# gabrielfnayres/new-vit

Measured on AMD Instinct MI355X. Metric: volumes_per_sec_mst_dinov2_fwd, higher is better.
Workload: dtype bf16; 1 GPU; MST-DINOv2 (DinoV2ClassifierSlice, ViT-S/14) forward, 4 volumes/GPU of 64x512x512 bf16 zero-padded to 518x518 (N=1370 tokens/slice); global_batch_volumes=4, slices=64, parallelism=single GPU, weights=synthetic (mst.synth seed 2), random init of the reference architecture

## Files before the change

new-vit_amd/csrc/k_gemm16_wreg.hip:

```cpp
#include <cstdlib>

#include "mst_common.h"

namespace {

constexpr int KD = GEMM16_WREG_TILE.bk, BN = GEMM16_WREG_TILE.bn, CH = GEMM16_WREG_TILE.bm;
constexpr int ROWB = KD * 2;
constexpr int SLOT = CH * ROWB;
constexpr int WREG_NSLOT = 4;
constexpr int NSLOT = WREG_NSLOT;
constexpr int STG_PITCH = ROWB + 16;
constexpr int STG_BYTES = CH * STG_PITCH;
constexpr int STG_OFF = NSLOT * SLOT;
constexpr int LDS_BYTES = STG_OFF + 2 * STG_BYTES;
constexpr int NKT = KD / 32;
constexpr int PPW = SLOT / 1024 / 8;
static_assert(NSLOT == 4, "the counted vmcnt table below is written for three chunks in flight");

#define WREG_RD(dst, base, imm) asm volatile("ds_read_b128 %0, %1 offset:%2" : "=v"(dst) : "v"(base), "n"(imm) : "memory")

template <typename T, bool BLK>
__global__ __launch_bounds__(512) __attribute__((amdgpu_waves_per_eu(2, 2))) void gemm16_wreg_kernel(
    const T* __restrict__ A, int64_t lda, const T* __restrict__ W, int64_t ldw, const float* __restrict__ bias, T* __restrict__ C,
    int64_t ldc, int M, int N, float col_scale, int scale_cols, int nchunks) {
    typedef typename V8<T>::type vec8;
    typedef __attribute__((ext_vector_type(4))) T out4;
    extern __shared__ __attribute__((aligned(16))) char smem[];
    const int lane = threadIdx.x & 63;
    const int wave = __builtin_amdgcn_readfirstlane(threadIdx.x >> 6);
    const int frow = lane & 15, kq = lane >> 4;

    const int xcd = blockIdx.x & 7, g = blockIdx.x >> 3, G = gridDim.x >> 3;
    const int tiles_n = N / BN;
    const int nt = g % tiles_n, jcu = g / tiles_n;
    const int c_nt = (G - nt + tiles_n - 1) / tiles_n;
    const int per_xcd = (nchunks + 7) >> 3;
    const int lo = xcd * per_xcd;
    const int hi = lo + per_xcd < nchunks ? lo + per_xcd : nchunks;
    const int n0 = nt * BN + wave * 48;
    const float cs = nt * BN < scale_cols ? col_scale : 1.f;

    vec8 w[3][NKT];
#pragma unroll
    for (int t = 0; t < 3; ++t) {
        const T* wr = W + (int64_t)(n0 + 12 * (frow >> 2) + 4 * t + (frow & 3)) * ldw + kq * 8;
#pragma unroll
        for (int kt = 0; kt < NKT; ++kt) w[t][kt] = *reinterpret_cast<const vec8*>(wr + kt * 32);
    }
    f32x4 b[3];
#pragma unroll
    for (int t = 0; t < 3; ++t) {
        b[t] = (f32x4){0.f, 0.f, 0.f, 0.f};
        if (bias) b[t] = *reinterpret_cast<const f32x4*>(bias + n0 + 12 * kq + 4 * t);
    }
#pragma unroll
    for (int t = 0; t < 3; ++t) {
        asm volatile("" : "+v"(b[t]));
#pragma unroll
        for (int kt = 0; kt < NKT; ++kt) asm volatile("" : "+v"(w[t][kt]));
    }

    unsigned dma_off[PPW];
#pragma unroll
    for (int u = 0; u < PPW; ++u) {
        const int o = (wave * PPW + u) * 1024 + lane * 16;
        const int r = o / ROWB;
        dma_off[u] = BLK ? (unsigned)o : (unsigned)(r * (int)lda * 2 + ((((o % ROWB) >> 4) ^ (r & 15)) << 4));
    }
    const int64_t chunk_bytes = BLK ? (int64_t)SLOT : (int64_t)CH * lda * 2;
    auto issue_piece = [&](int chunk, int slot, int u) {
        const char* base = reinterpret_cast<const char*>(A) + (int64_t)chunk * chunk_bytes;
        unsigned off = dma_off[u];
        const int valid = M - chunk * CH;
        if (!BLK && valid < CH) {
            const int o = (wave * PPW + u) * 1024 + lane * 16;
            int r = o / ROWB;
            const int ck = ((o % ROWB) >> 4) ^ (r & 15);
            r = r < valid ? r : valid - 1;
            off = (unsigned)(r * (int)lda * 2 + ck * 16);
        }
        __builtin_amdgcn_global_load_lds(GLB_PTR(base + off), LDS_PTR(smem + slot * SLOT + (wave * PPW + u) * 1024), 16, 0, 0);
    };

    int rb[4];
#pragma unroll
    for (int j = 0; j < 4; ++j) rb[j] = BLK ? (kq >> 1) * 1024 + (frow + 32 * (kq & 1)) * 16 : frow * ROWB + (((4 * j + kq) ^ frow) << 4);
    const int put_off = frow * STG_PITCH + wave * 96 + kq * 24;
    int fl_lds[3];
    unsigned fl_glb[3];
    int fl_row[3];
#pragma unroll
    for (int j = 0; j < 3; ++j) {
        const int q = lane + 64 * j;
        fl_row[j] = wave * 4 + q / 48;
        fl_lds[j] = fl_row[j] * STG_PITCH + (q % 48) * 16;
        fl_glb[j] = (unsigned)(fl_row[j] * (int)ldc * 2 + nt * BN * 2 + (q % 48) * 16);
    }
    f32x4 acc[2][3];
    auto put = [&](int it) {
        char* stg = smem + STG_OFF + (it & 1) * STG_BYTES + put_off;
#pragma unroll
        for (int mt = 0; mt < 2; ++mt)
#pragma unroll
            for (int t = 0; t < 3; ++t) {
                out4 pk;
#pragma unroll
                for (int i = 0; i < 4; ++i) pk[i] = (T)(acc[mt][t][i] * cs);
                *reinterpret_cast<out4*>(stg + mt * 16 * STG_PITCH + t * 8) = pk;
            }
    };
    auto flush_piece = [&](int chunk, int it, int j) {
        const char* stg = smem + STG_OFF + (it & 1) * STG_BYTES;
        char* cb = reinterpret_cast<char*>(C) + (int64_t)chunk * CH * ldc * 2;
        const int valid = M - chunk * CH;
        const u32x4 v = *reinterpret_cast<const u32x4*>(stg + fl_lds[j]);
        if (valid >= CH || fl_row[j] < valid) {
            __builtin_nontemporal_store(v, reinterpret_cast<u32x4*>(cb + fl_glb[j]));
        }
    };
    auto flush = [&](int chunk, int it) {
#pragma unroll
        for (int j = 0; j < 3; ++j) flush_piece(chunk, it, j);
    };

    int c = lo + jcu;
    if (c >= hi) return;
#pragma unroll
    for (int d = 0; d < NSLOT - 1; ++d)
        if (c + d * c_nt < hi) {
#pragma unroll
            for (int u = 0; u < PPW; ++u) issue_piece(c + d * c_nt, d, u);
        }

    int prev = -1, last_it = 0;
    for (int it = 0; c < hi; c += c_nt, ++it) {
        if (c + 2 * c_nt < hi) {
            if (it <= 1) asm volatile("s_waitcnt vmcnt(6)" ::: "memory");
            else if (it == 2) asm volatile("s_waitcnt vmcnt(9)" ::: "memory");
            else asm volatile("s_waitcnt vmcnt(12)" ::: "memory");
        } else {
            asm volatile("s_waitcnt vmcnt(0)" ::: "memory");
        }
        asm volatile("s_waitcnt lgkmcnt(0)\n\ts_barrier" ::: "memory");
        if (prev >= 0) flush(prev, it - 1);

        const int slot = it % NSLOT;
        const int nxt = c + (NSLOT - 1) * c_nt, nslot = (it + NSLOT - 1) % NSLOT;
        const bool more = nxt < hi;
        int rbs[4];
#pragma unroll
        for (int j = 0; j < 4; ++j) rbs[j] = rb[j] + slot * SLOT;
#pragma unroll
        for (int mt = 0; mt < 2; ++mt)
#pragma unroll
            for (int t = 0; t < 3; ++t) acc[mt][t] = b[t];

        u32x4 a[2][2];
        WREG_RD(a[0][0], rbs[0], 0);
        if constexpr (BLK) WREG_RD(a[0][1], rbs[0], 256);
        else WREG_RD(a[0][1], rbs[0], 16 * ROWB);
#pragma unroll
        for (int kt = 0; kt < NKT; ++kt) {
            const int cur = kt & 1;
            if (kt + 1 < NKT) {
                switch (kt + 1) {
#define WREG_NEXT(KN)                                                                  \
    case KN:                                                                           \
        if constexpr (BLK) {                                                           \
            WREG_RD(a[(KN) & 1][0], rbs[0], (KN) * 2048);                              \
            WREG_RD(a[(KN) & 1][1], rbs[0], (KN) * 2048 + 256);                        \
        } else {                                                                       \
            WREG_RD(a[(KN) & 1][0], rbs[(KN) & 3], ((KN) >> 2) * 256);                 \
            WREG_RD(a[(KN) & 1][1], rbs[(KN) & 3], 16 * ROWB + ((KN) >> 2) * 256);     \
        }                                                                              \
        break;
                    WREG_NEXT(1) WREG_NEXT(2) WREG_NEXT(3) WREG_NEXT(4) WREG_NEXT(5) WREG_NEXT(6)
                    WREG_NEXT(7) WREG_NEXT(8) WREG_NEXT(9) WREG_NEXT(10) WREG_NEXT(11)
#undef WREG_NEXT
                }
                asm volatile("s_waitcnt lgkmcnt(2)" : "+v"(a[cur][0]), "+v"(a[cur][1])::"memory");
            } else {
                asm volatile("s_waitcnt lgkmcnt(0)" : "+v"(a[cur][0]), "+v"(a[cur][1])::"memory");
            }
            const vec8 a0 = __builtin_bit_cast(vec8, a[cur][0]), a1 = __builtin_bit_cast(vec8, a[cur][1]);
#pragma unroll
            for (int t = 0; t < 3; ++t) {
                acc[0][t] = mfma16(w[t][kt], a0, acc[0][t]);
                acc[1][t] = mfma16(w[t][kt], a1, acc[1][t]);
            }
            if ((kt & 3) == 1) {
                __builtin_amdgcn_sched_barrier(0);
                if (more) issue_piece(nxt, nslot, kt >> 2);
                __builtin_amdgcn_sched_barrier(0);
            }
        }
        put(it);
        prev = c;
        last_it = it;
    }
    asm volatile("s_waitcnt lgkmcnt(0)\n\ts_barrier" ::: "memory");
    flush(prev, last_it);
}

template <typename T, bool BLK>
int launch_t(const gemm_args& g) {
    static mst_lds_once lds_once;
    auto kern = gemm16_wreg_kernel<T, BLK>;
    mst_allow_lds((const void*)kern, LDS_BYTES, &lds_once);
    const int nchunks = (int)((g.M + CH - 1) / CH);
    kern<<<dim3(mst_persistent_grid()), dim3(512), LDS_BYTES, g.s>>>((const T*)g.A, g.lda, (const T*)g.W, g.ldw, g.bias, (T*)g.C, g.ldc, (int)g.M,
                                                                      g.N, g.col_scale, g.scale_cols, nchunks);
    return mst_check_launch("gemm16_wreg");
}

}

int launch_gemm16_wreg(const gemm_args& g, int a_blocked) {
    if (a_blocked) {
        if (g.dt == MST_BF16) return launch_t<bf16_t, true>(g);
        if (g.dt == MST_F16) return launch_t<f16_t, true>(g);
    }
    if (g.dt == MST_BF16) return launch_t<bf16_t, false>(g);
    if (g.dt == MST_F16) return launch_t<f16_t, false>(g);
    mst_set_error("gemm16_wreg: bad operand dtype %d", g.dt);
    return MST_EINVAL;
}
```

new-vit_amd/mst/hip/__init__.py:

```python
from __future__ import annotations

import ctypes as C
import os
from pathlib import Path
from typing import Sequence, Optional, Tuple

import torch

_HERE = Path(__file__).resolve().parent
LIB_PATH = Path(os.environ.get("MST_HIP_LIB", _HERE / "libmst_hip.so"))

F32, F16, BF16, F8E4M3 = 0, 1, 2, 3
EPI_BIAS, EPI_BIAS_GELU, EPI_BIAS_RELU, EPI_RESIDUAL, EPI_RESIDUAL_RELU, EPI_BIAS_SWIGLU = 0, 1, 2, 3, 4, 5
FFN_MLP, FFN_SWIGLU = 0, 1
FUSION_TRANSFORMER, FUSION_LINEAR, FUSION_AVERAGE = 0, 1, 2

_DT = {torch.float32: F32, torch.float16: F16, torch.bfloat16: BF16}
TORCH_DT = {F32: torch.float32, F16: torch.float16, BF16: torch.bfloat16}
DT_NAMES = {"fp32": F32, "f32": F32, "float32": F32, "fp16": F16, "f16": F16, "float16": F16,
            "bf16": BF16, "bfloat16": BF16,
            "fp8": BF16, "f8": BF16, "fp8_e4m3": BF16}
FP8_NAMES = ("fp8", "f8", "fp8_e4m3")

_vp, _i, _i64, _f, _d, _sz = C.c_void_p, C.c_int, C.c_int64, C.c_float, C.c_double, C.c_size_t
# ... 117 lines not shown
    "mst_batchnorm_bwd_ordered": (_i, [_vp, _vp, _vp, _vp, _vp, _i64, _i, _vp, _vp, _vp, _vp, _sz, _vp]),
    "mst_col2im_nhwc_gather": (_i, [_vp, _i, _i, _i, _i, _i, _i, _i, _i, _i, _vp, _vp]),
    "mst_maxpool_bwd_nhwc_gather_workspace_bytes": (_sz, [_i, _i, _i, _i]),
    "mst_maxpool_bwd_nhwc_gather": (_i, [_vp, _vp, _i, _i, _i, _i, _vp, _vp, _sz, _vp]),
    "mst_pos_embed_interp_bwd_ordered_workspace_bytes": (_sz, [_i, _i, _i, _i]),
    "mst_pos_embed_interp_bwd_ordered": (_i, [_vp, _i, _i, _i, _i, _d, _vp, _vp, _sz, _vp]),
    "mst_znorm_ordered_workspace_bytes": (_sz, [_i64]),
    "mst_znorm_ordered": (_i, [_vp, _i64, _f, _f, _vp, _vp, _vp, _sz, _vp]),
    "mst_profiler_create": (_vp, []),
    "mst_profiler_destroy": (None, [_vp]),
    "mst_profiler_collect": (_i, [_vp, C.POINTER(C.c_double), C.POINTER(C.c_int64)]),
    "mst_kernel_kind_name": (C.c_char_p, [_i]),
}
K_COUNT = 10
ABI_VERSION = 300

_lib: Optional[C.CDLL] = None


def load() -> C.CDLL:
    global _lib
    if _lib is None:
        if not LIB_PATH.exists():
            raise RuntimeError(
                f"libmst_hip.so not found at {LIB_PATH}: build it with `python new-vit_amd/build.py` "
                "(hipcc --offload-arch=gfx950). There is no CPU / PyTorch fallback for the MST hot path.")
        lib = C.CDLL(str(LIB_PATH))
        for name, (res, args) in SIGNATURES.items():
            fn = getattr(lib, name)
            fn.restype, fn.argtypes = res, args
        if lib.mst_version() != ABI_VERSION:
            raise RuntimeError(f"{LIB_PATH} reports ABI version {lib.mst_version()}, this binding was written for {ABI_VERSION}: "
                               "rebuild with `python new-vit_amd/build.py --force`")
        _lib = lib
    return _lib


def last_error() -> str:
    return (load().mst_last_error() or b"").decode()


def _check(rc: int, what: str):
    if rc != 0:
        raise RuntimeError(f"{what} failed (status {rc}): {last_error()}")


def dt_of(t: torch.Tensor) -> int:
    try:
        return _DT[t.dtype]
    except KeyError:
        raise TypeError(f"unsupported dtype {t.dtype}") from None


def ptr(t: Optional[torch.Tensor]):
    return None if t is None else t.data_ptr()


def stream_of(t: torch.Tensor):
    return torch.cuda.current_stream(t.device).cuda_stream


def deterministic() -> bool:
    return torch.are_deterministic_algorithms_enabled()


def workspace(nbytes: int, device) -> Optional[torch.Tensor]:
    return torch.empty(int(nbytes), dtype=torch.uint8, device=device) if nbytes else None


def _call_ws(name: str, size_args, t: torch.Tensor, *args, sized_by: Optional[str] = None):
    lib = load()
    ws = workspace(getattr(lib, (sized_by or name) + "_workspace_bytes")(*size_args), t.device)
    _check(getattr(lib, name)(*args, ptr(ws), 0 if ws is None else ws.numel(), stream_of(t)), name)


def _dev(t: torch.Tensor, what: str):
    if not t.is_cuda:
        raise RuntimeError(f"{what}: tensor must live on a HIP device (got {t.device}); the MST kernels have no CPU path")
    if not t.is_contiguous():
        raise RuntimeError(f"{what}: tensor must be contiguous")


def layernorm(x: torch.Tensor, weight: torch.Tensor, bias: torch.Tensor, eps: float,
              out_dtype: torch.dtype = torch.float32) -> torch.Tensor:
    _dev(x, "layernorm")
    rows, cols = x.numel() // x.shape[-1], x.shape[-1]
    out = torch.empty(x.shape, dtype=out_dtype, device=x.device)
    _check(load().mst_layernorm(ptr(x), cols, ptr(weight), ptr(bias), ptr(out), _DT[out_dtype], cols, rows, cols,
                                eps, stream_of(x)), "mst_layernorm")
    return out


def gemm(a: torch.Tensor, w: torch.Tensor, bias: Optional[torch.Tensor], *, epilogue: int = EPI_BIAS,
         out: Optional[torch.Tensor] = None, out_dtype: Optional[torch.dtype] = None,
         gamma: Optional[torch.Tensor] = None, col_scale: float = 1.0, scale_cols: int = 0) -> torch.Tensor:
    _dev(a, "gemm")
    _dev(w, "gemm")
    M, K = a.shape
    N = w.shape[0]
    n_out = N // 2 if epilogue == EPI_BIAS_SWIGLU else N
    if out is None:
        out = torch.empty((M, n_out), dtype=out_dtype or a.dtype, device=a.device)
    _check(load().mst_gemm(ptr(a), dt_of(a), K, ptr(w), K, ptr(bias), ptr(out), dt_of(out), n_out, M, N, K, epilogue,
                           ptr(gamma), col_scale, scale_cols, stream_of(a)), "mst_gemm")
    return out


F8_MAX = 448.0


def quantize_weight_fp8(w: torch.Tensor) -> Tuple[torch.Tensor, float]:
    w = w.detach().to(torch.float32)
    amax = float(w.abs().max())
    scale = amax / F8_MAX if amax > 0 else 1.0
    q = (w / scale).clamp(-F8_MAX, F8_MAX).to(torch.float8_e4m3fn)
    return q.view(torch.uint8).contiguous(), scale


def quantize_fp8(x: torch.Tensor, amax: Optional[torch.Tensor] = None) -> Tuple[torch.Tensor, torch.Tensor]:
    _dev(x, "quantize_fp8")
    if amax is None:
        amax = torch.zeros(1, dtype=torch.float32, device=x.device)
    out = torch.empty(x.shape, dtype=torch.uint8, device=x.device)
    _check(load().mst_quantize_fp8(ptr(x), dt_of(x), x.numel(), ptr(amax), ptr(out), stream_of(x)), "mst_quantize_fp8")
    return out, amax


def gemm_fp8(a8: torch.Tensor, a_amax: torch.Tensor, w8: torch.Tensor, w_scale: float, bias: Optional[torch.Tensor], *,
             epilogue: int = EPI_BIAS, out: Optional[torch.Tensor] = None, out_dtype: torch.dtype = torch.float32,
             gamma: Optional[torch.Tensor] = None, col_scale: float = 1.0, scale_cols: int = 0,
             c_amax: Optional[torch.Tensor] = None) -> torch.Tensor:
    _dev(a8, "gemm_fp8")
    _dev(w8, "gemm_fp8")
    M, K = a8.shape
    N = w8.shape[0]
    if out is None:
        out = torch.empty((M, N), dtype=torch.uint8 if c_amax is not None else out_dtype, device=a8.device)
    cdt = F8E4M3 if c_amax is not None else dt_of(out)
    _check(load().mst_gemm_fp8(ptr(a8), K, ptr(w8), K, ptr(bias), ptr(a_amax), w_scale, ptr(out), cdt, N, M, N, K,
                               epilogue, ptr(gamma), col_scale, scale_cols, ptr(c_amax), stream_of(a8)), "mst_gemm_fp8")
    return out


def layernorm_fp8(x: torch.Tensor, gamma: Optional[torch.Tensor], beta: Optional[torch.Tensor], eps: float,
                  amax: torch.Tensor) -> torch.Tensor:
    _dev(x, "layernorm_fp8")
    rows, cols = x.shape
    out = torch.empty((rows, cols), dtype=torch.uint8, device=x.device)
    _check(load().mst_layernorm_fp8(ptr(x), cols, ptr(gamma), ptr(beta), ptr(out), cols, rows, cols, eps, ptr(amax),
                                    stream_of(x)), "mst_layernorm_fp8")
    return out


def attention(qkv: torch.Tensor, n_seq: int, N: int, heads: int, head_dim: int = 64) -> torch.Tensor:
    _dev(qkv, "attention")
    out = torch.empty((n_seq * N, heads * head_dim), dtype=qkv.dtype, device=qkv.device)
    _check(load().mst_attention(ptr(qkv), dt_of(qkv), n_seq, N, heads, head_dim, ptr(out), stream_of(qkv)), "mst_attention")
    return out


def attention_cls_probs(qkv: torch.Tensor, n_seq: int, N: int, heads: int, head_dim: int = 64) -> torch.Tensor:
    _dev(qkv, "attention_cls_probs")
    out = torch.empty((n_seq, heads, N), dtype=torch.float32, device=qkv.device)
    _check(load().mst_attention_cls_probs(ptr(qkv), dt_of(qkv), n_seq, N, heads, head_dim, ptr(out), stream_of(qkv)),
           "mst_attention_cls_probs")
    return out


def attention_probs_full(qkv: torch.Tensor, n_seq: int, N: int, heads: int, head_dim: int = 64) -> torch.Tensor:
    _dev(qkv, "attention_probs_full")
    out = torch.empty((n_seq, heads, N, N), dtype=torch.float32, device=qkv.device)
    _check(load().mst_attention_probs_full(ptr(qkv), dt_of(qkv), n_seq, N, heads, head_dim, ptr(out), stream_of(qkv)),
           "mst_attention_probs_full")
    return out


def _train_attn_args(qkv16: torch.Tensor, n_seq: int, N: int, heads: int, head_dim: int, what: str):
    _dev(qkv16, what)
    if qkv16.dtype not in (torch.bfloat16, torch.float16):
        raise TypeError(f"{what}: qkv16 must be bf16 or fp16 (got {qkv16.dtype})")
    if n_seq < 1 or N < 1 or heads < 1 or tuple(qkv16.shape) != (n_seq * N, 3 * heads * head_dim):
        raise ValueError(f"{what}: qkv16 {tuple(qkv16.shape)} is not [n_seq*N, 3*heads*head_dim] for n_seq={n_seq} N={N} heads={heads} "
                         f"head_dim={head_dim}")


def _f32_like(t: torch.Tensor, shape, dev, what: str, name: str):
    _dev(t, what)
    if t.dtype != torch.float32 or tuple(t.shape) != tuple(shape) or t.device != dev:
        raise ValueError(f"{what}: {name} must be fp32 {tuple(shape)} on {dev} (got {t.dtype} {tuple(t.shape)} on {t.device})")


def attention_train_fwd(qkv16: torch.Tensor, n_seq: int, N: int, heads: int, head_dim: int = 64,
                        out_dtype: torch.dtype = torch.float32) -> Tuple[torch.Tensor, torch.Tensor]:
    _train_attn_args(qkv16, n_seq, N, heads, head_dim, "attention_train_fwd")
    if out_dtype not in (torch.float32, qkv16.dtype):
        raise ValueError(f"attention_train_fwd: out_dtype must be fp32 or qkv16's {qkv16.dtype} (got {out_dtype})")
    out = torch.empty((n_seq * N, heads * head_dim), dtype=out_dtype, device=qkv16.device)
    lse = torch.empty((n_seq, heads, N), dtype=torch.float32, device=qkv16.device)
    lib = load()
    fn, what = (lib.mst_attention_train_fwd, "mst_attention_train_fwd") if out_dtype == torch.float32 else \
               (lib.mst_attention_train_fwd16, "mst_attention_train_fwd16")
    _check(fn(ptr(qkv16), dt_of(qkv16), n_seq, N, heads, head_dim, ptr(out), ptr(lse), stream_of(qkv16)), what)
    return out, lse


def attention_train_bwd(qkv16: torch.Tensor, out: torch.Tensor, dout: torch.Tensor, lse: torch.Tensor, n_seq: int, N: int, heads: int,
                        dq_scale: float = 1.0, head_dim: int = 64, dqkv: Optional[torch.Tensor] = None) -> torch.Tensor:
    what = "attention_train_bwd"
    _train_attn_args(qkv16, n_seq, N, heads, head_dim, what)
    dev = qkv16.device
    out16 = out.dtype == qkv16.dtype
    if out16:
        _dev(out, what)
        if tuple(out.shape) != (n_seq * N, heads * head_dim) or out.device != dev:
            raise ValueError(f"{what}: out must be [{n_seq * N}, {heads * head_dim}] on {dev} (got {tuple(out.shape)} on {out.device})")
    else:
        _f32_like(out, (n_seq * N, heads * head_dim), dev, what, "out")
    _f32_like(dout, (n_seq * N, heads * head_dim), dev, what, "dout")
    _f32_like(lse, (n_seq, heads, N), dev, what, "lse")
    if dqkv is None:
        dqkv = torch.empty((n_seq * N, 3 * heads * head_dim), dtype=torch.float32, device=dev)
    _f32_like(dqkv, (n_seq * N, 3 * heads * head_dim), dev, what, "dqkv")
    _call_ws("mst_attention_train_bwd16" if out16 else "mst_attention_train_bwd", (n_seq, N, heads, head_dim), qkv16,
             ptr(qkv16), dt_of(qkv16), ptr(out), ptr(dout), ptr(lse), n_seq, N, heads, head_dim, dq_scale, ptr(dqkv),
             sized_by="mst_attention_train_bwd")
    return dqkv


def pos_embed_interp(pos_patch: torch.Tensor, M: int, gh: int, gw: int, offset: float = 0.1,
                     antialias: bool = False) -> torch.Tensor:
    _dev(pos_patch, "pos_embed_interp")
    E = pos_patch.shape[-1]
    out = torch.empty((gh * gw, E), dtype=torch.float32, device=pos_patch.device)
    _check(load().mst_pos_embed_interp(ptr(pos_patch), M, E, gh, gw, offset, 1 if antialias else 0, ptr(out), stream_of(pos_patch)),
           "mst_pos_embed_interp")
    return out


def patch_embed(vol: torch.Tensor, wp: torch.Tensor, bias: torch.Tensor, prefix: torch.Tensor,
                pos_patch: torch.Tensor) -> torch.Tensor:
    _dev(vol, "patch_embed")
    n, H, W = vol.shape
    E = wp.shape[0]
    n_prefix = prefix.shape[0]
    N = n_prefix + (H // 14) * (W // 14)
    x = torch.empty((n, N, E), dtype=torch.float32, device=vol.device)
    _check(load().mst_patch_embed(ptr(vol), dt_of(vol), n, H, W, ptr(wp), dt_of(wp), ptr(bias), ptr(prefix), n_prefix,
                                  ptr(pos_patch), E, ptr(x), stream_of(vol)), "mst_patch_embed")
    return x


def slices2rgb(vol: torch.Tensor) -> torch.Tensor:
    _dev(vol, "slices2rgb")
    B, C, D, H, W = vol.shape
    assert C == 1, "More than one channel"
    Dp = (D + 2) // 3 * 3
    out = torch.empty((B * Dp // 3, 3, H, W), dtype=vol.dtype, device=vol.device)
    _check(load().mst_slices2rgb(ptr(vol), dt_of(vol), B, D, H, W, ptr(out), stream_of(vol)), "mst_slices2rgb")
    return out


def mlp_fused(x: torch.Tensor, wpack: torch.Tensor, b1f: torch.Tensor, b2f: torch.Tensor,
              xn_out: Optional[torch.Tensor], dtype: torch.dtype, eps: float = 1e-6):
    _dev(x, "mlp_fused")
    M, E = x.shape
    _check(load().mst_mlp_fused(ptr(x), ptr(xn_out), _DT[dtype], ptr(wpack), ptr(b1f), ptr(b2f), M, E, eps,
                                stream_of(x)), "mst_mlp_fused")


def block_fused(x: torch.Tensor, attn_out: torch.Tensor, proj_pack: torch.Tensor, proj_bf: torch.Tensor, wpack: torch.Tensor,
                b1f: torch.Tensor, b2f: torch.Tensor, xn_out: Optional[torch.Tensor], eps: float = 1e-6,
                scratch: Optional[torch.Tensor] = None):
    _dev(x, "block_fused")
    _dev(attn_out, "block_fused")
    M, E = x.shape
    if scratch is None:
        scratch = torch.empty(int(load().mst_block_fused_scratch_bytes()), dtype=torch.uint8, device=x.device)
    _check(load().mst_block_fused(ptr(x), ptr(attn_out), ptr(xn_out), dt_of(attn_out), ptr(proj_pack), ptr(proj_bf), ptr(wpack),
                                  ptr(b1f), ptr(b2f), ptr(scratch), scratch.numel(), M, E, eps, stream_of(x)), "mst_block_fused")


def block_fused_s(x: torch.Tensor, attn_out: torch.Tensor, block_seq: torch.Tensor, b1f: torch.Tensor, proj_bf: torch.Tensor,
                  b2f: torch.Tensor, xn_out: Optional[torch.Tensor], eps: float = 1e-6, layout: int = 0):
    _dev(x, "block_fused_s")
    _dev(attn_out, "block_fused_s")
    M, E = x.shape
    _check(load().mst_block_fused_s(ptr(x), ptr(attn_out), ptr(xn_out), dt_of(attn_out), ptr(block_seq), ptr(b1f), ptr(proj_bf),
                                    ptr(b2f), M, E, eps, layout, stream_of(x)), "mst_block_fused_s")


LAYOUT_X_IN_IMAGE, LAYOUT_X_OUT_IMAGE, LAYOUT_ACT_BLOCKED = 1, 2, 4


def to_blocked16(a: torch.Tensor) -> torch.Tensor:
    M, Cn = a.shape
    return a.reshape(M // 32, 32, Cn // 16, 2, 8).permute(0, 2, 3, 1, 4).contiguous().reshape(M, Cn)


def from_blocked16(a: torch.Tensor) -> torch.Tensor:
    M, Cn = a.shape
    return a.reshape(M // 32, Cn // 16, 2, 32, 8).permute(0, 3, 1, 2, 4).contiguous().reshape(M, Cn)


def to_image32(a: torch.Tensor) -> torch.Tensor:
    M, Cn = a.shape
    return a.reshape(M // 32, 32, Cn // 8, 2, 4).permute(0, 2, 3, 1, 4).contiguous().reshape(M, Cn)


def from_image32(a: torch.Tensor) -> torch.Tensor:
    M, Cn = a.shape
    return a.reshape(M // 32, Cn // 8, 2, 32, 4).permute(0, 3, 1, 2, 4).contiguous().reshape(M, Cn)


def pack_block_seq(proj_w, proj_b, ls1, fc1_w, fc1_b, fc2_w, fc2_b, ln_w, ln_b, ls2, dtype: torch.dtype):
    dev = proj_w.device
    wp = proj_w.float()
    pbf = proj_b.float().clone()
    if ls1 is not None:
        wp = wp * ls1.float()[:, None]
        pbf = pbf * ls1.float()
    w1 = fc1_w.float() * ln_w.float()[None, :]
    b1f = fc1_b.float() + (fc1_w.float() * ln_b.float()[None, :]).sum(dim=1)
    w2 = fc2_w.float()
    b2f = fc2_b.float().clone()
    if ls2 is not None:
        w2 = w2 * ls2.float()[:, None]
        b2f = b2f * ls2.float()
    ar = lambda n: torch.arange(n, device=dev)
    lane = ar(64)
    m, h = (lane & 31)[None, None, :, None], (lane >> 5)[None, None, :, None]
    t, p, e = ar(12)[:, None, None, None], ar(2)[None, :, None, None], ar(8)[None, None, None, :]
    k8 = 16 * p + 8 * (e >> 2) + 4 * h + (e & 3)
    rows_t = (32 * t + m).expand(12, 2, 64, 8)
    kp = (16 * p + 8 * h + e).expand(12, 2, 64, 8)
    proj = torch.stack([wp[rows_t, 32 * j + kp] for j in range(12)])
    cols1 = (32 * t + k8).expand(12, 2, 64, 8)
    rows1 = m.expand(12, 2, 64, 8)
    w1c = torch.stack([w1[32 * c + rows1, cols1] for c in range(48)])
    k2 = k8.expand(12, 2, 64, 8)
    w2c = torch.stack([w2[rows_t, 32 * c + k2] for c in range(48)])
    proj, w1c, w2c = proj.reshape(12, -1), w1c.reshape(48, -1), w2c.reshape(48, -1)
    seq = [proj, w1c[0:1]]
    inter = torch.stack([w1c[1:48], w2c[0:47]], dim=1).reshape(94, -1)
    seq += [inter, w2c[47:48]]
    block_seq = torch.cat(seq, dim=0).to(dtype).contiguous()
    assert block_seq.shape == (108, 12288)
    return block_seq, b1f.contiguous(), pbf.contiguous(), b2f.contiguous()


def _w2_row_order(dev):
    R = torch.arange(384, device=dev)
    t, i = R >> 4, R & 15
    nphys = 32 * (t >> 1) + 8 * (i >> 2) + 4 * (t & 1) + (i & 3)
    cidx = torch.arange(4, device=dev)[None, :] ^ ((-(R >> 2)) & 3)[:, None]
    return R, nphys, cidx


def pack_proj(proj_w, proj_b, ls1, dtype: torch.dtype):
    dev = proj_w.device
    w = proj_w.float()
    b = proj_b.float().clone()
    if ls1 is not None:
        w = w * ls1.float()[:, None]
        b = b * ls1.float()
    R, nphys, cidx = _w2_row_order(dev)
    wc = w[nphys].view(384, 12, 4, 8).permute(1, 0, 2, 3)
    img = wc[:, R[:, None], cidx, :]
    return img.reshape(12, -1).to(dtype).contiguous(), b.contiguous()


def pack_mlp(fc1_w, fc1_b, fc2_w, fc2_b, ln_w, ln_b, ls2, dtype: torch.dtype):
    dev = fc1_w.device
    w1f = fc1_w.float() * ln_w.float()[None, :]
    b1f = fc1_b.float() + (fc1_w.float() * ln_b.float()[None, :]).sum(dim=1)
    b2f = fc2_b.float().clone()
    if ls2 is not None:
        fc2_w = fc2_w.float() * ls2.float()[:, None]
        b2f = b2f * ls2.float()
    ar = lambda n: torch.arange(n, device=dev)
    w1c = w1f.view(48, 32, 12, 4, 8).permute(0, 2, 1, 3, 4)
    fh = (-(ar(32) >> 2)) & 3
    cidx = ar(4)[None, :] ^ fh[:, None]
    w1img = w1c[:, :, ar(32)[:, None], cidx, :]
    p = ar(32); c = p >> 3; j = p & 7
    phys = torch.where(j < 4, 4 * c + j, 16 + 4 * c + j - 4)
    R = ar(384); t = R >> 4; i = R & 15
    nphys = 32 * (t >> 1) + 8 * (i >> 2) + 4 * (t & 1) + (i & 3)
    w2p = fc2_w.float().view(384, 48, 32)[:, :, phys][nphys]
    w2c = w2p.permute(1, 0, 2).reshape(48, 384, 4, 8)
    fR = (-(R >> 2)) & 3
    cidxR = ar(4)[None, :] ^ fR[:, None]
    w2img = w2c[:, R[:, None], cidxR, :]
    wpack = torch.cat([w1img.reshape(48, -1), w2img.reshape(48, -1)], dim=1).to(dtype).contiguous()
    b1p = torch.zeros(1536 + 32, device=dev, dtype=torch.float32)
    b1p[:1536] = b1f
    return wpack, b1p, b2f.contiguous()


def swiglu_hidden(embed_dim: int) -> int:
    return (int(4 * embed_dim * 2 / 3) + 7) // 8 * 8


def swiglu_group(dtype: torch.dtype) -> int:
    return 32 if dtype == torch.float32 else 16


def pack_swiglu(w12, b12, w3, dtype: torch.dtype):
    H2, E = w12.shape
    H = H2 // 2
    if H2 != 2 * H or tuple(b12.shape) != (H2,) or tuple(w3.shape) != (E, H):
        raise ValueError(f"pack_swiglu: w12 {tuple(w12.shape)}, b12 {tuple(b12.shape)}, w3 {tuple(w3.shape)} are not [2H, E], [2H], [E, H]")
    G = swiglu_group(dtype)
    Hp = (H + 63) // 64 * 64
    dev = w12.device
    wg = torch.zeros((2, Hp, E), dtype=torch.float32, device=dev)
    wg[:, :H] = w12.detach().float().view(2, H, E)
    bg = torch.zeros((2, Hp), dtype=torch.float32, device=dev)
    bg[:, :H] = b12.detach().float().view(2, H)
    w12p = wg.view(2, Hp // G, G, E).permute(1, 0, 2, 3).reshape(2 * Hp, E).to(dtype).contiguous()
    b12p = bg.view(2, Hp // G, G).permute(1, 0, 2).reshape(2 * Hp).contiguous()
    w3p = torch.zeros((E, Hp), dtype=torch.float32, device=dev)
    w3p[:, :H] = w3.detach().float()
    return w12p, b12p, w3p.to(dtype).contiguous()


def vit_workspace_bytes(w: VitWeights, H: int, W: int, chunk: int) -> int:
    return int(load().mst_vit_workspace_bytes(C.byref(w), H, W, chunk))


def vit_encode(w: VitWeights, vol: torch.Tensor, cls_out: torch.Tensor, cls_probs: Optional[torch.Tensor],
               n_layers_probs: int, chunk: int, ws: torch.Tensor, full_probs: Optional[torch.Tensor] = None):
    _dev(vol, "vit_encode")
    n, H, W = vol.shape
    _check(load().mst_vit_encode(C.byref(w), ptr(vol), dt_of(vol), n, H, W, ptr(cls_out), ptr(cls_probs),
                                 ptr(full_probs), n_layers_probs, chunk, ptr(ws), ws.numel() * ws.element_size(),
                                 stream_of(vol)), "mst_vit_encode")


def fusion_workspace_bytes(w: FusionWeights, B: int, D: int) -> int:
    return int(load().mst_fusion_workspace_bytes(C.byref(w), B, D))


def slice_fusion(w: FusionWeights, emb: torch.Tensor, B: int, D: int, mask: Optional[torch.Tensor],
                 features: torch.Tensor, logits: Optional[torch.Tensor], slice_probs: Optional[torch.Tensor],
                 ws: torch.Tensor):
    _dev(emb, "slice_fusion")
    _check(load().mst_slice_fusion(C.byref(w), ptr(emb), B, D, ptr(mask), ptr(features), ptr(logits), ptr(slice_probs),
                                   ptr(ws), ws.numel() * ws.element_size(), stream_of(emb)), "mst_slice_fusion")


def attention_readout(cls_probs_last: Optional[torch.Tensor], slice_probs: Optional[torch.Tensor], B: int, D: int,
                      heads: int, N: int, num_registers: int, sheads: int, plane: Optional[torch.Tensor],
                      slice_attn: Optional[torch.Tensor], maps: Optional[torch.Tensor]):
    t = cls_probs_last if cls_probs_last is not None else slice_probs
    _check(load().mst_attention_readout(ptr(cls_probs_last), ptr(slice_probs), B, D, heads, N, num_registers, sheads,
                                        ptr(plane), ptr(slice_attn), ptr(maps), stream_of(t)), "mst_attention_readout")


def saliency_accumulate(maps: torch.Tensor, slice_attn: Optional[torch.Tensor], gh: int, gw: int, flip_mask: int,
                        lowres: torch.Tensor, slice_acc: Optional[torch.Tensor], accumulate: bool):
    _dev(maps, "saliency_accumulate")
    D, heads, Np = maps.shape
    _check(load().mst_saliency_accumulate(ptr(maps), ptr(slice_attn), D, heads, gh, gw, Np, flip_mask, 1 if accumulate else 0,
                                          ptr(lowres), ptr(slice_acc), stream_of(maps)), "mst_saliency_accumulate")


def saliency_upsample(lowres: torch.Tensor, size, scale: float = 1.0) -> torch.Tensor:
    _dev(lowres, "saliency_upsample")
    D, gh, gw = lowres.shape
    Dout, H, W = (int(v) for v in size)
    out = torch.empty((Dout, H, W), dtype=torch.float32, device=lowres.device)
    _check(load().mst_saliency_upsample(ptr(lowres), D, gh, gw, float(scale), Dout, H, W, ptr(out), stream_of(lowres)),
           "mst_saliency_upsample")
    return out


def liere_rotation(vars_: Sequence[torch.Tensor]) -> torch.Tensor:
    v = torch.stack([t.detach().float().reshape(t.shape[0], t.shape[1]) for t in vars_]).contiguous()
    _dev(v, "liere_rotation")
    nb, m, P = v.shape
    n = int(round((1 + (1 + 8 * m) ** 0.5) / 2))
    if n * (n - 1) // 2 != m:
        raise ValueError(f"liere_rotation: {m} parameters per block is not n(n-1)/2")
    R = torch.empty((nb * n, nb * n), dtype=torch.float32, device=v.device)
    _check(load().mst_liere_rotation(ptr(v), nb, n, P, ptr(R), stream_of(v)), "mst_liere_rotation")
    return R


def attention_rollout(maps: Sequence[torch.Tensor]) -> torch.Tensor:
    m0 = maps[0]
    _dev(m0, "attention_rollout")
    N = m0.shape[-1]
    for m in maps:
        if m.dtype != torch.float32 or tuple(m.shape) != tuple(m0.shape) or m.shape[-2] != N or not m.is_contiguous():
            raise ValueError("attention_rollout: maps must be contiguous fp32 [..., N, N] tensors of one shape")
    batch = m0.numel() // (N * N)
    out = torch.empty_like(m0)
    tmp = torch.empty_like(m0) if len(maps) > 2 else None
    arr = (_vp * len(maps))(*[ptr(m) for m in maps])
    _check(load().mst_attention_rollout(arr, len(maps), batch, N, ptr(out), ptr(tmp), stream_of(m0)),
           "mst_attention_rollout")
    return out


def gemm_ex(A: torch.Tensor, B: torch.Tensor, C: torch.Tensor, M: int, N: int, K: int, sa, sb, sc, nb=(1, 1),
            ba=(0, 0), bb=(0, 0), bc=(0, 0), alpha: float = 1.0, beta: float = 0.0, offs=(0, 0, 0)):
    st = (_i64 * 12)(sa[0], sa[1], sb[0], sb[1], sc[0], sc[1], ba[0], ba[1], bb[0], bb[1], bc[0], bc[1])
    _check(load().mst_gemm_ex(A.data_ptr() + 4 * offs[0], B.data_ptr() + 4 * offs[1], C.data_ptr() + 4 * offs[2], M, N, K, st,
                              nb[0], nb[1], alpha, beta, stream_of(C)), "mst_gemm_ex")
    return C


def cvt16(x: torch.Tensor, dtype: torch.dtype, *, transpose: bool = False, rows_pad: Optional[int] = None, scale: float = 1.0) -> torch.Tensor:
    _dev(x, "cvt16")
    rows, cols = x.shape
    if transpose:
        rp = rows_pad or rows
        out = torch.empty((cols, rp), dtype=dtype, device=x.device)
        _check(load().mst_cvt16(ptr(x), cols, rows, cols, scale, ptr(out), dt_of(out), rp, 1, rp, stream_of(x)), "mst_cvt16")
        return out
    out = torch.empty((rows, cols), dtype=dtype, device=x.device)
    _check(load().mst_cvt16(ptr(x), cols, rows, cols, scale, ptr(out), dt_of(out), cols, 0, rows, stream_of(x)), "mst_cvt16")
    return out


def gemm16_splitk(a: torch.Tensor, w: torch.Tensor, splits: int) -> torch.Tensor:
    _dev(a, "gemm16_splitk")
    _dev(w, "gemm16_splitk")
    M, K = a.shape
    N = w.shape[0]
    part = torch.empty((splits, M, N), dtype=torch.float32, device=a.device)
    _check(load().mst_gemm16_splitk(ptr(a), dt_of(a), K, ptr(w), K, ptr(part), N, M, N, K, splits, M * N, stream_of(a)), "mst_gemm16_splitk")
    return part


def rope_rows(qkv: torch.Tensor, L: int, heads: int, hd: int, freqs: torch.Tensor, sign: float = 1.0) -> torch.Tensor:
    _dev(qkv, "rope_rows")
    _check(load().mst_rope_rows(ptr(qkv), qkv.shape[0], L, heads, hd, ptr(freqs), sign, stream_of(qkv)), "mst_rope_rows")
    return qkv


def softmax_rows(S: torch.Tensor, mask: Optional[torch.Tensor], rows_per_batch: int):
    L = S.shape[-1]
    _check(load().mst_softmax_rows(ptr(S), ptr(mask), S.numel() // L, L, rows_per_batch, stream_of(S)), "mst_softmax_rows")
    return S


def softmax_rows_bwd(P: torch.Tensor, dP: torch.Tensor, scale: float = 1.0):
    L = P.shape[-1]
    _check(load().mst_softmax_rows_bwd(ptr(P), ptr(dP), P.numel() // L, L, scale, stream_of(P)), "mst_softmax_rows_bwd")
    return dP


def layernorm_rows(x: torch.Tensor, x_stride: int, rows: int, cols: int, weight, bias, eps: float) -> torch.Tensor:
    out = torch.empty((rows, cols), dtype=torch.float32, device=x.device)
    _check(load().mst_layernorm(ptr(x), x_stride, ptr(weight), ptr(bias), ptr(out), F32, cols, rows, cols, eps, stream_of(x)),
           "mst_layernorm")
    return out


def layernorm_bwd(x, x_stride, gamma, dy, dy_stride, dres, dres_stride, dx, dx_stride, dgamma, dbeta, rows, cols, eps):
    if deterministic():
        _call_ws("mst_layernorm_bwd_ordered", (rows, cols), x, ptr(x), x_stride, ptr(gamma), ptr(dy), dy_stride, ptr(dres), dres_stride,
                 ptr(dx), dx_stride, ptr(dgamma), ptr(dbeta), rows, cols, eps)
        return
    _check(load().mst_layernorm_bwd(ptr(x), x_stride, ptr(gamma), ptr(dy), dy_stride, ptr(dres), dres_stride, ptr(dx), dx_stride,
                                    ptr(dgamma), ptr(dbeta), rows, cols, eps, stream_of(x)), "mst_layernorm_bwd")


def act_fwd(h: torch.Tensor, kind: int) -> torch.Tensor:
    y = torch.empty_like(h)
    if h.dtype == torch.float32:
        _check(load().mst_act_fwd(ptr(h), ptr(y), h.numel(), kind, stream_of(h)), "mst_act_fwd")
    else:
        _check(load().mst_act_fwd16(ptr(h), ptr(y), dt_of(h), h.numel(), kind, stream_of(h)), "mst_act_fwd16")
    return y


def act_bwd(h: torch.Tensor, dy: torch.Tensor, kind: int) -> torch.Tensor:
    if h.dtype == torch.float32:
        _check(load().mst_act_bwd(ptr(h), ptr(dy), h.numel(), kind, stream_of(h)), "mst_act_bwd")
    else:
        _check(load().mst_act_bwd16(ptr(h), dt_of(h), ptr(dy), h.numel(), kind, stream_of(h)), "mst_act_bwd16")
    return dy


def swiglu_fwd(x12: torch.Tensor) -> torch.Tensor:
    _dev(x12, "swiglu_fwd")
    rows, H2 = x12.shape
    if H2 % 2:
        raise ValueError("swiglu_fwd: x12 must have an even number of columns")
    h = torch.empty((rows, H2 // 2), dtype=x12.dtype, device=x12.device)
    if x12.dtype == torch.float32:
        _check(load().mst_swiglu_fwd(ptr(x12), ptr(h), rows, H2 // 2, stream_of(x12)), "mst_swiglu_fwd")
    else:
        _check(load().mst_swiglu_fwd16(ptr(x12), ptr(h), dt_of(x12), rows, H2 // 2, stream_of(x12)), "mst_swiglu_fwd16")
    return h


def swiglu_bwd(x12: torch.Tensor, dh: torch.Tensor) -> torch.Tensor:
    _dev(x12, "swiglu_bwd")
    _dev(dh, "swiglu_bwd")
    rows, H2 = x12.shape
    if dh.dtype != torch.float32 or tuple(dh.shape) != (rows, H2 // 2) or H2 % 2 or dh.device != x12.device:
        raise ValueError("swiglu_bwd: dh must be fp32 [rows, H] on x12's device for x12 [rows, 2H]")
    dx = torch.empty((rows, H2), dtype=torch.float32, device=x12.device)
# ... 393 lines not shown
```

Before: 162.3 volumes/s.

## Balance wreg GEMM work across CUs with tail segments over all N-tiles

Replaces the fixed per-CU assignment of one N-tile with a strided chunk range by a share scheme. Most CUs keep one N-tile over a strided range of full rounds, while the leftover CUs each take contiguous slices of the remaining chunks across every N-tile. This targets load imbalance when the CU count per XCD is not a multiple of the N-tile count. In exchange, tail CUs reload weight registers and restart the prefetch pipeline per segment, and a Python helper mirrors the schedule.

```diff
diff --git a/new-vit_amd/csrc/k_gemm16_wreg.hip b/new-vit_amd/csrc/k_gemm16_wreg.hip
--- a/new-vit_amd/csrc/k_gemm16_wreg.hip
+++ b/new-vit_amd/csrc/k_gemm16_wreg.hip
@@ -19,6 +19,25 @@
 
 #define WREG_RD(dst, base, imm) asm volatile("ds_read_b128 %0, %1 offset:%2" : "=v"(dst) : "v"(base), "n"(imm) : "memory")
 
+struct wreg_seg { int nt, c0, c1, step; };
+struct wreg_shares {
+    int T, q, nf, rem, S;
+    __device__ wreg_shares(int G, int T_, int n) : T(T_) {
+        q = G / T;
+        const int r = G - q * T, k = (T * n + G - 1) / G;
+        nf = q * k < n ? q * k : n;
+        rem = n - nf;
+        S = r ? (T * rem + r - 1) / r : 0;
+    }
+    __device__ int nseg(int g) const { return g < q * T ? 1 : T; }
+    __device__ wreg_seg segment(int g, int s) const {
+        if (g < q * T) return {g % T, g / T, nf, q};
+        const int f = g - q * T;
+        const int a = f * S > s * rem ? f * S : s * rem, e = (f + 1) * S < (s + 1) * rem ? (f + 1) * S : (s + 1) * rem;
+        return {s, nf + a - s * rem, nf + e - s * rem, 1};
+    }
+};
+
 template <typename T, bool BLK>
 __global__ __launch_bounds__(512) __attribute__((amdgpu_waves_per_eu(2, 2))) void gemm16_wreg_kernel(
     const T* __restrict__ A, int64_t lda, const T* __restrict__ W, int64_t ldw, const float* __restrict__ bias, T* __restrict__ C,
@@ -32,33 +51,11 @@
 
     const int xcd = blockIdx.x & 7, g = blockIdx.x >> 3, G = gridDim.x >> 3;
     const int tiles_n = N / BN;
-    const int nt = g % tiles_n, jcu = g / tiles_n;
-    const int c_nt = (G - nt + tiles_n - 1) / tiles_n;
     const int per_xcd = (nchunks + 7) >> 3;
     const int lo = xcd * per_xcd;
     const int hi = lo + per_xcd < nchunks ? lo + per_xcd : nchunks;
-    const int n0 = nt * BN + wave * 48;
-    const float cs = nt * BN < scale_cols ? col_scale : 1.f;
-
-    vec8 w[3][NKT];
-#pragma unroll
-    for (int t = 0; t < 3; ++t) {
-        const T* wr = W + (int64_t)(n0 + 12 * (frow >> 2) + 4 * t + (frow & 3)) * ldw + kq * 8;
-#pragma unroll
-        for (int kt = 0; kt < NKT; ++kt) w[t][kt] = *reinterpret_cast<const vec8*>(wr + kt * 32);
-    }
-    f32x4 b[3];
-#pragma unroll
-    for (int t = 0; t < 3; ++t) {
-        b[t] = (f32x4){0.f, 0.f, 0.f, 0.f};
-        if (bias) b[t] = *reinterpret_cast<const f32x4*>(bias + n0 + 12 * kq + 4 * t);
-    }
-#pragma unroll
-    for (int t = 0; t < 3; ++t) {
-        asm volatile("" : "+v"(b[t]));
-#pragma unroll
-        for (int kt = 0; kt < NKT; ++kt) asm volatile("" : "+v"(w[t][kt]));
-    }
+    if (hi <= lo) return;
+    const wreg_shares sh(G, tiles_n, hi - lo);
 
     unsigned dma_off[PPW];
 #pragma unroll
@@ -94,8 +91,12 @@
         const int q = lane + 64 * j;
         fl_row[j] = wave * 4 + q / 48;
         fl_lds[j] = fl_row[j] * STG_PITCH + (q % 48) * 16;
-        fl_glb[j] = (unsigned)(fl_row[j] * (int)ldc * 2 + nt * BN * 2 + (q % 48) * 16);
-    }
+        fl_glb[j] = (unsigned)(fl_row[j] * (int)ldc * 2 + (q % 48) * 16);
+    }
+    vec8 w[3][NKT];
+    f32x4 b[3];
+    float cs = 1.f;
+    int col_bytes = 0;
     f32x4 acc[2][3];
     auto put = [&](int it) {
         char* stg = smem + STG_OFF + (it & 1) * STG_BYTES + put_off;
@@ -111,7 +112,7 @@
     };
     auto flush_piece = [&](int chunk, int it, int j) {
         const char* stg = smem + STG_OFF + (it & 1) * STG_BYTES;
-        char* cb = reinterpret_cast<char*>(C) + (int64_t)chunk * CH * ldc * 2;
+        char* cb = reinterpret_cast<char*>(C) + (int64_t)chunk * CH * ldc * 2 + col_bytes;
         const int valid = M - chunk * CH;
         const u32x4 v = *reinterpret_cast<const u32x4*>(stg + fl_lds[j]);
         if (valid >= CH || fl_row[j] < valid) {
@@ -123,47 +124,73 @@
         for (int j = 0; j < 3; ++j) flush_piece(chunk, it, j);
     };
 
-    int c = lo + jcu;
-    if (c >= hi) return;
-#pragma unroll
-    for (int d = 0; d < NSLOT - 1; ++d)
-        if (c + d * c_nt < hi) {
-#pragma unroll
-            for (int u = 0; u < PPW; ++u) issue_piece(c + d * c_nt, d, u);
-        }
-
-    int prev = -1, last_it = 0;
-    for (int it = 0; c < hi; c += c_nt, ++it) {
-        if (c + 2 * c_nt < hi) {
-            if (it <= 1) asm volatile("s_waitcnt vmcnt(6)" ::: "memory");
-            else if (it == 2) asm volatile("s_waitcnt vmcnt(9)" ::: "memory");
-            else asm volatile("s_waitcnt vmcnt(12)" ::: "memory");
-        } else {
-            asm volatile("s_waitcnt vmcnt(0)" ::: "memory");
-        }
-        asm volatile("s_waitcnt lgkmcnt(0)\n\ts_barrier" ::: "memory");
-        if (prev >= 0) flush(prev, it - 1);
-
-        const int slot = it % NSLOT;
-        const int nxt = c + (NSLOT - 1) * c_nt, nslot = (it + NSLOT - 1) % NSLOT;
-        const bool more = nxt < hi;
-        int rbs[4];
-#pragma unroll
-        for (int j = 0; j < 4; ++j) rbs[j] = rb[j] + slot * SLOT;
-#pragma unroll
-        for (int mt = 0; mt < 2; ++mt)
-#pragma unroll
-            for (int t = 0; t < 3; ++t) acc[mt][t] = b[t];
-
-        u32x4 a[2][2];
-        WREG_RD(a[0][0], rbs[0], 0);
-        if constexpr (BLK) WREG_RD(a[0][1], rbs[0], 256);
-        else WREG_RD(a[0][1], rbs[0], 16 * ROWB);
-#pragma unroll
-        for (int kt = 0; kt < NKT; ++kt) {
-            const int cur = kt & 1;
-            if (kt + 1 < NKT) {
-                switch (kt + 1) {
+    const int nseg = sh.nseg(g);
+    for (int s = 0; s < nseg; ++s) {
+        const wreg_seg sg = sh.segment(g, s);
+        if (sg.c0 >= sg.c1) continue;
+        const int c_nt = sg.step, end = lo + sg.c1;
+        const int n0 = sg.nt * BN + wave * 48;
+        cs = sg.nt * BN < scale_cols ? col_scale : 1.f;
+        col_bytes = sg.nt * BN * 2;
+
+#pragma unroll
+        for (int t = 0; t < 3; ++t) {
+            const T* wr = W + (int64_t)(n0 + 12 * (frow >> 2) + 4 * t + (frow & 3)) * ldw + kq * 8;
+#pragma unroll
+            for (int kt = 0; kt < NKT; ++kt) w[t][kt] = *reinterpret_cast<const vec8*>(wr + kt * 32);
+        }
+#pragma unroll
+        for (int t = 0; t < 3; ++t) {
+            b[t] = (f32x4){0.f, 0.f, 0.f, 0.f};
+            if (bias) b[t] = *reinterpret_cast<const f32x4*>(bias + n0 + 12 * kq + 4 * t);
+        }
+#pragma unroll
+        for (int t = 0; t < 3; ++t) {
+            asm volatile("" : "+v"(b[t]));
+#pragma unroll
+            for (int kt = 0; kt < NKT; ++kt) asm volatile("" : "+v"(w[t][kt]));
+        }
+
+        int c = lo + sg.c0;
+#pragma unroll
+        for (int d = 0; d < NSLOT - 1; ++d)
+            if (c + d * c_nt < end) {
+#pragma unroll
+                for (int u = 0; u < PPW; ++u) issue_piece(c + d * c_nt, d, u);
+            }
+
+        int prev = -1, last_it = 0;
+        for (int it = 0; c < end; c += c_nt, ++it) {
+            if (c + 2 * c_nt < end) {
+                if (it <= 1) asm volatile("s_waitcnt vmcnt(6)" ::: "memory");
+                else if (it == 2) asm volatile("s_waitcnt vmcnt(9)" ::: "memory");
+                else asm volatile("s_waitcnt vmcnt(12)" ::: "memory");
+            } else {
+                asm volatile("s_waitcnt vmcnt(0)" ::: "memory");
+            }
+            asm volatile("s_waitcnt lgkmcnt(0)\n\ts_barrier" ::: "memory");
+            if (prev >= 0) flush(prev, it - 1);
+
+            const int slot = it % NSLOT;
+            const int nxt = c + (NSLOT - 1) * c_nt, nslot = (it + NSLOT - 1) % NSLOT;
+            const bool more = nxt < end;
+            int rbs[4];
+#pragma unroll
+            for (int j = 0; j < 4; ++j) rbs[j] = rb[j] + slot * SLOT;
+#pragma unroll
+            for (int mt = 0; mt < 2; ++mt)
+#pragma unroll
+                for (int t = 0; t < 3; ++t) acc[mt][t] = b[t];
+
+            u32x4 a[2][2];
+            WREG_RD(a[0][0], rbs[0], 0);
+            if constexpr (BLK) WREG_RD(a[0][1], rbs[0], 256);
+            else WREG_RD(a[0][1], rbs[0], 16 * ROWB);
+#pragma unroll
+            for (int kt = 0; kt < NKT; ++kt) {
+                const int cur = kt & 1;
+                if (kt + 1 < NKT) {
+                    switch (kt + 1) {
 #define WREG_NEXT(KN)                                                                  \
     case KN:                                                                           \
         if constexpr (BLK) {                                                           \
@@ -174,32 +201,33 @@
             WREG_RD(a[(KN) & 1][1], rbs[(KN) & 3], 16 * ROWB + ((KN) >> 2) * 256);     \
         }                                                                              \
         break;
-                    WREG_NEXT(1) WREG_NEXT(2) WREG_NEXT(3) WREG_NEXT(4) WREG_NEXT(5) WREG_NEXT(6)
-                    WREG_NEXT(7) WREG_NEXT(8) WREG_NEXT(9) WREG_NEXT(10) WREG_NEXT(11)
+                        WREG_NEXT(1) WREG_NEXT(2) WREG_NEXT(3) WREG_NEXT(4) WREG_NEXT(5) WREG_NEXT(6)
+                        WREG_NEXT(7) WREG_NEXT(8) WREG_NEXT(9) WREG_NEXT(10) WREG_NEXT(11)
 #undef WREG_NEXT
+                    }
+                    asm volatile("s_waitcnt lgkmcnt(2)" : "+v"(a[cur][0]), "+v"(a[cur][1])::"memory");
+                } else {
+                    asm volatile("s_waitcnt lgkmcnt(0)" : "+v"(a[cur][0]), "+v"(a[cur][1])::"memory");
                 }
-                asm volatile("s_waitcnt lgkmcnt(2)" : "+v"(a[cur][0]), "+v"(a[cur][1])::"memory");
-            } else {
-                asm volatile("s_waitcnt lgkmcnt(0)" : "+v"(a[cur][0]), "+v"(a[cur][1])::"memory");
-            }
-            const vec8 a0 = __builtin_bit_cast(vec8, a[cur][0]), a1 = __builtin_bit_cast(vec8, a[cur][1]);
-#pragma unroll
-            for (int t = 0; t < 3; ++t) {
-                acc[0][t] = mfma16(w[t][kt], a0, acc[0][t]);
-                acc[1][t] = mfma16(w[t][kt], a1, acc[1][t]);
-            }
-            if ((kt & 3) == 1) {
-                __builtin_amdgcn_sched_barrier(0);
-                if (more) issue_piece(nxt, nslot, kt >> 2);
-                __builtin_amdgcn_sched_barrier(0);
-            }
-        }
-        put(it);
-        prev = c;
-        last_it = it;
-    }
-    asm volatile("s_waitcnt lgkmcnt(0)\n\ts_barrier" ::: "memory");
-    flush(prev, last_it);
+                const vec8 a0 = __builtin_bit_cast(vec8, a[cur][0]), a1 = __builtin_bit_cast(vec8, a[cur][1]);
+#pragma unroll
+                for (int t = 0; t < 3; ++t) {
+                    acc[0][t] = mfma16(w[t][kt], a0, acc[0][t]);
+                    acc[1][t] = mfma16(w[t][kt], a1, acc[1][t]);
+                }
+                if ((kt & 3) == 1) {
+                    __builtin_amdgcn_sched_barrier(0);
+                    if (more) issue_piece(nxt, nslot, kt >> 2);
+                    __builtin_amdgcn_sched_barrier(0);
+                }
+            }
+            put(it);
+            prev = c;
+            last_it = it;
+        }
+        asm volatile("s_waitcnt lgkmcnt(0)\n\ts_barrier" ::: "memory");
+        flush(prev, last_it);
+    }
 }
 
 template <typename T, bool BLK>
diff --git a/new-vit_amd/mst/hip/__init__.py b/new-vit_amd/mst/hip/__init__.py
--- a/new-vit_amd/mst/hip/__init__.py
+++ b/new-vit_amd/mst/hip/__init__.py
@@ -443,6 +443,23 @@
     return a.reshape(M // 32, Cn // 16, 2, 32, 8).permute(0, 3, 1, 2, 4).contiguous().reshape(M, Cn)
 
 
+def wreg_segments(G: int, T: int, n: int) -> list:
+    q = G // T
+    r, k = G - q * T, -(-T * n // G)
+    nf = min(n, q * k)
+    rem = n - nf
+    S = -(-T * rem // r) if r else 0
+    out = []
+    for g in range(G):
+        if g < q * T:
+            segs = [(g % T, range(g // T, nf, q))]
+        else:
+            f = g - q * T
+            segs = [(s, range(nf + max(f * S, s * rem) - s * rem, nf + min((f + 1) * S, (s + 1) * rem) - s * rem)) for s in range(T)]
+        out.append([(t, c) for t, c in segs if len(c)])
+    return out
+
+
 def to_image32(a: torch.Tensor) -> torch.Tensor:
     M, Cn = a.shape
     return a.reshape(M // 32, 32, Cn // 8, 2, 4).permute(0, 2, 3, 1, 4).contiguous().reshape(M, Cn)
```

New measurement: 162.5 volumes/s, median of 6. Within noise of the previous version (+0.1%).
